# tum-vision/mono_dataset_code

Hardware: AMD Instinct MI355X
Metric: Mpix/s photometric+FOV undistort, 1280x1024 gray (higher is better)
Workload: dtype f32

## Files before the change

### mono_dataset_code_amd/build.py

```python
import os
import shutil
import subprocess
import time
import sys

PKG = os.path.dirname(os.path.abspath(__file__))
ROOT = os.path.dirname(PKG)
CSRC = os.path.join(PKG, "csrc")
HOST = os.path.join(CSRC, "host")
INC = os.path.join(ROOT, "include")
EIGEN_STUB = os.path.join(INC, "mono_dataset_code", "compat")

LIB_HIP = os.path.join(PKG, "libmdc_hip.so")
LIB_HOST = os.path.join(PKG, "libmdc_host.so")

HIP_SOURCES = [os.path.join(CSRC, f) for f in ("mdc_kernels.hip", "mdc_vcal.hip", "mdc_jpeg.hip", "mdc_capi.hip", "mdc_plan.hip", "mdc_host_calls.hip",
                                                "mdc_pipeline.hip", "mdc_placement.hip", "mdc_rcal.hip")]
HIP_DEPS = HIP_SOURCES + [os.path.join(CSRC, "mdc_exports.map"), os.path.join(CSRC, "mdc_internal.h"), os.path.join(CSRC, "mdc_ctx.h"), os.path.join(CSRC, "mdc_build_config.h"), os.path.join(CSRC, "fov_point_model.h"), os.path.join(CSRC, "minmax_first.h"), os.path.join(CSRC, "placement_classes.h"), os.path.join(CSRC, "xcd_placement.h"), os.path.join(INC, "mdc_hip.h")]
HOST_SOURCES = [os.path.join(HOST, f) for f in (
    "fov_undistorter.cpp", "photometric_undistorter.cpp", "gray_png.cpp", "host_device.cpp", "mdc_host_capi.cpp",
    "image_codecs.cpp", "image_codecs_png.cpp", "image_codecs_jpeg.cpp", "image_codecs_jpeg_stream.cpp", "zip_reader.cpp", "image_pool.cpp", "frame_source.cpp", "decode_pool.cpp",
    "prefetch_cache.cpp", "device_lanes.cpp", "batch_run.cpp", "dataset_reader.cpp")]
HOST_DEPS = HOST_SOURCES + [os.path.join(HOST, "mdc_host_exports.map"), os.path.join(HOST, "gray_png.h"), os.path.join(HOST, "host_device.h"),
                            os.path.join(HOST, "image_codecs.h"), os.path.join(HOST, "image_codecs_internal.h"), os.path.join(HOST, "image_codecs_jpeg.h"), os.path.join(HOST, "zip_reader.h"),
                            os.path.join(HOST, "frame_source.h"), os.path.join(HOST, "decode_pool.h"), os.path.join(HOST, "prefetch_cache.h"),
                            os.path.join(HOST, "device_lanes.h"), os.path.join(HOST, "batch_run.h"), os.path.join(CSRC, "png_inflate_core.h"),
                            os.path.join(INC, "mono_dataset_code", "BenchmarkDatasetReader.h"),
                            os.path.join(INC, "mdc_hip.h"), os.path.join(INC, "mdc_host.h"), os.path.join(INC, "mdc_lens.h"),
                            os.path.join(INC, "mdc_lensinv.h"), os.path.join(CSRC, "lens_inverse_model.h"),
                            os.path.join(CSRC, "lens_point_model.h"), os.path.join(CSRC, "fov_point_model.h"),
                            os.path.join(INC, "mono_dataset_code", "FOVUndistorter.h"),
                            os.path.join(INC, "mono_dataset_code", "PhotometricUndistorter.h"),
                            os.path.join(INC, "mono_dataset_code", "ExposureImage.h"),
                            os.path.join(INC, "mono_dataset_code", "MdcBind.h")]

HIP_FLAGS = ["--offload-arch=gfx950", "-O3", "-std=c++17", "-ffp-contract=off", "-fPIC", "-shared",
             "-fno-fast-math", "-fvisibility=hidden", "-fvisibility-inlines-hidden", "-Wall", "-Wno-unused-function"]
HOST_FLAGS = ["-O2", "-std=c++11", "-ffp-contract=off", "-fPIC", "-shared", "-fvisibility=hidden", "-fvisibility-inlines-hidden", "-Wall"]
HOST_EXPORT_MAP = os.path.join(HOST, "mdc_host_exports.map")
EXPORT_MAP = os.path.join(CSRC, "mdc_exports.map")
RECIPE = os.path.abspath(__file__)


def _stale(target, deps):
    if not os.path.exists(target):
        return True
    t = os.path.getmtime(target)
    return any(os.path.getmtime(d) > t for d in deps)


def _run(cmd):
    r = subprocess.run(cmd, stdout=subprocess.PIPE, stderr=subprocess.STDOUT, text=True)
    if r.returncode != 0:
        sys.stderr.write(r.stdout)
        raise RuntimeError("build failed: " + " ".join(cmd))
    return r.stdout


def hipcc():
    for c in (os.environ.get("HIPCC"), shutil.which("hipcc"), "/opt/rocm/bin/hipcc"):
        if c and os.path.exists(c):
            return c
    raise RuntimeError("hipcc not found")


def eigen_include():
    for d in ("/usr/include/eigen3", "/usr/local/include/eigen3"):
        if os.path.exists(os.path.join(d, "Eigen", "Core")):
            return d
    return EIGEN_STUB

# ... 382 lines not shown
```

### mono_dataset_code_amd/csrc/mdc_capi.hip

```cpp
#include "mdc_ctx.h"

using namespace mdc;


namespace mdc {

static thread_local std::string g_create_err;
static thread_local std::string t_err, t_err_other;
static thread_local const mdc_ctx* t_err_ctx = nullptr;

int fail(mdc_ctx* c, int code, const char* fmt, ...) {
  char buf[512];
  va_list ap;
  va_start(ap, fmt);
  vsnprintf(buf, sizeof buf, fmt, ap);
  va_end(ap);
  if (c) {
    {
      std::lock_guard<std::mutex> lk(c->err_mu);
      c->err = buf;
    }
    t_err = buf;
    t_err_ctx = c;
  } else {
// ... 898 lines not shown
  if (n < 0 || (n > 0 && (!d_vignette || !d_out)) || ((uintptr_t)d_out & 1) || ((uintptr_t)d_vignette & 3))
    return fail(c, MDC_ERR_ARG, "mdc_vcal_vignette_u16_device: bad argument");
  ReadLock lk(c->mu);
  DeviceGuard dg(c->device);
  MDC_HIP(c, launch_vcal_vignette_u16(d_vignette, n, d_out, (hipStream_t)stream));
  return MDC_OK;
} MDC_CATCH(c)

int mdc_vcal_solve_device(mdc_ctx* c, const float* d_images, const float* d_p2x, const float* d_p2y, int n_images, int w, int h,
                          int n_plane, float* d_plane_color, float* d_vignette_factor, int max_iterations, int outlier_th,
                          double* er_out, void* stream) try {
  if (!c) return MDC_ERR_ARG;
  if (!d_plane_color || !d_vignette_factor || max_iterations < 0 || outlier_th < 0 || outlier_th > 46340)
    return fail(c, MDC_ERR_ARG, "mdc_vcal_solve_device: bad argument");
  if (max_iterations == 0) return MDC_OK;
  mdc_vcal_index* index = nullptr;
  int rc = mdc_vcal_index_create(c, d_images, d_p2x, d_p2y, n_images, w, h, n_plane, stream, &index);
  if (rc != MDC_OK) return rc;
  ReadLock lk(c->mu);
  DeviceGuard dg(c->device);
  hipStream_t s = (hipStream_t)stream;
  float *d_ff = nullptr, *d_fc = nullptr, *d_tt = nullptr, *d_ct = nullptr;
  double* d_er = nullptr;
  const size_t plane_bytes = (size_t)std::max(n_plane, 1) * sizeof(float), img_bytes = (size_t)w * h * sizeof(float);
  const size_t er_bytes = (size_t)max_iterations * 4 * sizeof(double);
  auto done = [&](int code) {
    (void)hipStreamSynchronize(s);
    for (void* p : {(void*)d_ff, (void*)d_fc, (void*)d_tt, (void*)d_ct, (void*)d_er}) (void)hipFree(p);
    mdc_vcal_index_destroy(index);
    return code;
  };
#define MDC_SOLVE(call_)                                                  \
  do {                                                                    \
    hipError_t e_ = (call_);                                              \
    if (e_ != hipSuccess) return done(fail(c, MDC_ERR_HIP, "%s: %s", #call_, hipGetErrorString(e_))); \
  } while (0)
  MDC_SOLVE(hipMalloc(&d_ff, plane_bytes));
  MDC_SOLVE(hipMalloc(&d_fc, plane_bytes));
  MDC_SOLVE(hipMalloc(&d_tt, img_bytes));
  MDC_SOLVE(hipMalloc(&d_ct, img_bytes));
  MDC_SOLVE(hipMalloc(&d_er, er_bytes));
  for (int it = 0; it < max_iterations; it++) {
    const int oth2 = it < max_iterations / 2 ? 10000 * 10000 : outlier_th * outlier_th;
    MDC_SOLVE(launch_vcal_plane_step(d_images, d_p2x, d_p2y, n_images, w, h, n_plane, d_plane_color, d_vignette_factor, oth2, d_ff,
                                     d_fc, d_er + 4 * it, s));
    MDC_SOLVE(mdc::launch_vcal_vignette_step_indexed(index->ix, d_plane_color, d_vignette_factor, oth2, d_tt, d_ct, d_er + 4 * it + 2,
                                                     c->d_vcal_max + (c->vcal_max_next++ % mdc_ctx::kVcalMaxWords), s));
  }
  if (er_out) MDC_SOLVE(hipMemcpyAsync(er_out, d_er, er_bytes, hipMemcpyDeviceToHost, s));
#undef MDC_SOLVE
  return done(MDC_OK);
} MDC_CATCH(c)

int mdc_tune_device(mdc_ctx* c, const uint8_t* d_in, float* d_out, int64_t nframes, unsigned flags, void* stream,
                    mdc_tune_result* result) try {
  if (!c) return MDC_ERR_ARG;
  if (!d_in || !d_out || nframes <= 0) return fail(c, MDC_ERR_ARG, "mdc_tune_device: bad argument");
  WriteLock lk(c->mu);
  DeviceGuard dg(c->device);
  if (!(flags & MDC_RECTIFY) || !c->valid_remap) return fail(c, MDC_ERR_STATE, "mdc_tune_device: needs a remap and MDC_RECTIFY");
  hipStream_t s = (hipStream_t)stream;
  static const TileShape shapes[] = {{128, 16}, {64, 32}, {128, 32}};
  static const int fpbs[] = {32, 64, 96, 128};
  hipEvent_t e0, e1;
  MDC_HIP(c, hipEventCreate(&e0));
  MDC_HIP(c, hipEventCreate(&e1));
  float best = 1e30f;
  int bw = 0, bh = 0, bf = 0, tried = 0;
  int rc = MDC_OK;
  const int caller_fpb = c->opt_fpb;
  for (const TileShape& sh : shapes) {
    c->opt_tile_w = sh.w;
    c->opt_tile_h = sh.h;
    if (hipDeviceSynchronize() != hipSuccess) {
      rc = fail(c, MDC_ERR_HIP, "mdc_tune_device: hipDeviceSynchronize failed");
      break;
    }
    if ((rc = plan_tiles(c)) != MDC_OK) break;
    if (!c->plan[0].tiled) continue;
    for (int fpb : fpbs) {
      c->opt_fpb = fpb;
      float ms[5];
      bool ok = true;
      for (int k = 0; k < 7 && ok; k++) {
        if (k >= 2) ok = hipEventRecord(e0, s) == hipSuccess;
        ok = ok && enqueue_process(c, d_in, d_out, nframes, flags, s) == MDC_OK;
        if (k >= 2) ok = ok && hipEventRecord(e1, s) == hipSuccess && hipEventSynchronize(e1) == hipSuccess &&
                         hipEventElapsedTime(&ms[k - 2], e0, e1) == hipSuccess;
      }
      if (!ok) continue;
      std::sort(ms, ms + 5);
      tried++;
      if (ms[2] < best) {
        best = ms[2];
        bw = sh.w;
        bh = sh.h;
        bf = fpb;
      }
    }
  }
  (void)hipEventDestroy(e0);
  (void)hipEventDestroy(e1);
  (void)hipDeviceSynchronize();
  c->opt_tile_w = bw;
  c->opt_tile_h = bh;
  c->opt_fpb = caller_fpb;
  c->tuned_fpb = bf;
  c->tuned_min_frames = bf ? std::max<int64_t>(nframes / 4, (int64_t)bf * 8) : 0;
  const int rc2 = plan_tiles(c);
  if (rc == MDC_OK) rc = rc2;
  if (result) {
    result->tile_w = bw;
    result->tile_h = bh;
    result->frames_per_block = bf;
    result->ms = tried ? best : 0.f;
    result->candidates = tried;
  }
  return rc;
} MDC_CATCH(c)

int mdc_tune_placement_device(mdc_ctx* c, const uint8_t* const* d_in, int n_in, float* const* d_out, int n_out, int64_t nframes, unsigned flags,
                              void* stream, int* best_in, int* best_out, float* ms_out) try {
  if (!c) return MDC_ERR_ARG;
  if (!d_in || !d_out || n_in < 1 || n_out < 1 || (int64_t)n_in * n_out > 256 || nframes <= 0 || !best_in || !best_out)
    return fail(c, MDC_ERR_ARG, "mdc_tune_placement_device: bad argument");
  for (int k = 0; k < n_in; k++)
    if (!d_in[k]) return fail(c, MDC_ERR_ARG, "mdc_tune_placement_device: input candidate %d is NULL", k);
  for (int k = 0; k < n_out; k++)
    if (!d_out[k]) return fail(c, MDC_ERR_ARG, "mdc_tune_placement_device: output candidate %d is NULL", k);
  ReadLock lk(c->mu);
  DeviceGuard dg(c->device);
  hipStream_t s = (hipStream_t)stream;
  hipEvent_t e0, e1;
  MDC_HIP(c, hipEventCreate(&e0));
  if (hipEventCreate(&e1) != hipSuccess) {
    (void)hipEventDestroy(e0);
    return fail(c, MDC_ERR_HIP, "hipEventCreate failed");
  }
  int rc = MDC_OK, bi = 0, bo = 0;
  float best = 1e30f;
  for (int i = 0; i < n_in && rc == MDC_OK; i++)
    for (int j = 0; j < n_out && rc == MDC_OK; j++) {
      float ms[5] = {0, 0, 0, 0, 0};
      for (int k = 0; k < 7 && rc == MDC_OK; k++) {
        bool ok = k < 2 || hipEventRecord(e0, s) == hipSuccess;
        if (ok) rc = enqueue_process(c, d_in[i], d_out[j], nframes, flags, s);
        if (rc != MDC_OK) break;
        if (k >= 2) ok = ok && hipEventRecord(e1, s) == hipSuccess && hipEventSynchronize(e1) == hipSuccess && hipEventElapsedTime(&ms[k - 2], e0, e1) == hipSuccess;
        if (!ok) rc = fail(c, MDC_ERR_HIP, "mdc_tune_placement_device: timing a launch failed");
      }
      if (rc != MDC_OK) break;
      std::sort(ms, ms + 5);
      if (ms_out) ms_out[(size_t)i * n_out + j] = ms[2];
      if (ms[2] < best) {
        best = ms[2];
        bi = i;
        bo = j;
      }
    }
  (void)hipStreamSynchronize(s);
  (void)hipEventDestroy(e0);
  (void)hipEventDestroy(e1);
  *best_in = bi;
  *best_out = bo;
  return rc;
} MDC_CATCH(c)

int mdc_describe_launch(mdc_ctx* c, unsigned flags, int pyramid_levels, char* buf, size_t cap) try {
// ... 158 lines not shown
```

### mono_dataset_code_amd/csrc/mdc_ctx.h

```cpp
#pragma once
#include "../../include/mdc_hip.h"
#include "mdc_internal.h"

#include <algorithm>
#include <atomic>
#include <chrono>
#include <cmath>
#include <condition_variable>
#include <cstdarg>
#include <cstdio>
#include <cstdlib>
#include <cstring>
#include <limits>
#include <map>
#include <mutex>
#include <new>
#include <shared_mutex>
#include <string>
#include <vector>

struct mdc_ctx {
  int device = 0;
  std::shared_timed_mutex mu;
  mutable std::mutex err_mu;
// ... 103 lines not shown
  std::atomic<unsigned> vcal_max_next{0};

};
using ReadLock = std::shared_lock<std::shared_timed_mutex>;
using WriteLock = std::unique_lock<std::shared_timed_mutex>;

namespace mdc {

int fail(mdc_ctx* c, int code, const char* fmt, ...);

#define MDC_HIP(c, call)                                                                      \
  do {                                                                                        \
    hipError_t e_ = (call);                                                                   \
    if (e_ != hipSuccess) return fail((c), MDC_ERR_HIP, "%s: %s", #call, hipGetErrorString(e_)); \
  } while (0)

struct DeviceGuard {
  int prev = -1;
  explicit DeviceGuard(int dev) {
    if (hipGetDevice(&prev) != hipSuccess) prev = -1;
    if (prev != dev) (void)hipSetDevice(dev);
    else prev = -1;
  }
  ~DeviceGuard() {
    if (prev >= 0) (void)hipSetDevice(prev);
  }
};

#define MDC_CATCH(c_)                                                                    \
  catch (const std::bad_alloc&) {                                                        \
    return fail((c_), MDC_ERR_NOMEM, "out of host memory");                              \
  }                                                                                      \
  catch (const std::exception& e_) {                                                     \
    return fail((c_), MDC_ERR_HIP, "unexpected exception: %s", e_.what());               \
  }                                                                                      \
  catch (...) {                                                                          \
    return fail((c_), MDC_ERR_HIP, "unexpected exception");                              \
  }

void normalise(const mdc_ctx* c, unsigned flags, bool& g, bool& v, bool& o);
const float* lut_for(const mdc_ctx* c, bool g, bool o);
int frames_per_block(const mdc_ctx* c, int64_t nframes, int blocks_per_group, int target_wgs = 4800);
TilePlan tile_plan(const mdc_ctx* c, int which);
RemapArgs remap_args(const mdc_ctx* c, const float* lut, const float* vinv);
int enqueue_process(mdc_ctx* c, const uint8_t* d_in, float* d_out, int64_t nframes, unsigned flags, hipStream_t s, float* const* pyr = nullptr,
                    bool* pyr_done = nullptr);
int enqueue_pyramid_gradients(mdc_ctx* c, const uint8_t* d_in, float* d_base, int levels, float* const* d_levels, float* const* d_dI,
                              float* const* d_abs_squared_grad, int64_t nframes, unsigned flags, int chunk_frames, hipStream_t s);
int enqueue_undistort_f32(mdc_ctx* c, const float* d_in, float* d_out, int64_t nframes, hipStream_t s);
DistortModel distort_model(const mdc_fov_model* f);

int plan_tiles(mdc_ctx* c);
void free_plan(mdc_ctx* c);

void maybe_pin(mdc_ctx* c, int role, const void* p, size_t bytes);
void unpin_all(mdc_ctx* c);
const void* device_view_raw(const mdc_ctx* c, const void* p, size_t bytes);
template <class T>
T* device_view(const mdc_ctx* c, T* p, size_t bytes) {
  return (T*)device_view_raw(c, (const void*)p, bytes);
}
bool one_host_allocation(const void* p, size_t bytes);
int ensure_stage(mdc_ctx* c, mdc_ctx::HostSlot* h, size_t in_bytes, size_t out_bytes);

struct SlotLease {
  mdc_ctx* c;
  mdc_ctx::HostSlot* s = nullptr;
  explicit SlotLease(mdc_ctx* ctx, bool wait = true);
  bool in_flight = true;
  void drained() { in_flight = false; }
  ~SlotLease();
  SlotLease(const SlotLease&) = delete;
  SlotLease& operator=(const SlotLease&) = delete;
};

}
```

### mono_dataset_code_amd/csrc/mdc_internal.h

```cpp
#pragma once
#include <hip/hip_runtime.h>
#include <stdint.h>

#include "fov_point_model.h"
#include "mdc_build_config.h"
#include "xcd_placement.h"

namespace mdc {

struct TileShape {
  int w, h;
};
constexpr TileShape kTileShapes[] = {{64, 16}, {64, 32}, {64, 60}, {64, 64}, {128, 16}, {128, 32}};
constexpr bool tile_shape_ok(int w, int h) {
  for (const TileShape& t : kTileShapes)
    if (t.w == w && t.h == h) return true;
  return false;
}
constexpr int tile_rpt(int w, int h) { return w >= 320 ? 8 : 4; }
constexpr int tile_threads(int w, int h) { return w * h / tile_rpt(w, h); }
constexpr int kTileMaxChunks = 3;
constexpr int kTileMaxChunksF32 = 4;
constexpr int kLutRep = MDC_EXP_LUT_REP;
constexpr uint32_t kOutside = 0xfffffff0u;

struct RemapArgs {
  const float* lut;
  const float* vinv;
  const float* rx;
  const float* ry;
  int in_w, in_h, out_w, out_h;
};

struct TilePlan {
  const uint32_t* d_chunks;
  const int* d_nch;
  const uint32_t* d_taps;
  const int* d_order;
  int n_blocks;
  int n_tiles, tiles_x;
  int tile_w;
  int tile_h;
  int chunk_cap;
  int win_bytes;
  int nbuf;
  bool has_black;
  bool interleave;
  bool taper = true;
  bool rotate = false;
};

constexpr int kStripTileW = 128, kStripTileH = 8;
constexpr int kStripChunkCap = 128;
constexpr int kStripWaves = MDC_EXP_STRIP_WAVES;
struct StripPlan {
  const uint32_t* d_chunks;
  const int* d_nch;
  const uint32_t* d_taps;
  const int* d_order;
  int n_blocks, n_tiles, tiles_x;
  int win_bytes;
  int passes;
  int nbuf;
  bool interleave;
  bool rotate = false;
};
#if MDC_EXP_STRIP_FAKE_GRAD
extern float* g_fake_grad_dI;
extern float* g_fake_grad_abs;
#endif
hipError_t launch_remap_strip_u8(const uint8_t* d_in, float* d_out, const RemapArgs& a, const StripPlan& p, int64_t nframes, int fpb,
                                 hipStream_t s, float* d_l1 = nullptr, float* d_l2 = nullptr, float* d_l3 = nullptr);
size_t strip_lds_bytes(int win_bytes, int nbuf, int waves);

hipError_t launch_unmap(const uint8_t* d_in, float* d_out, const float* d_lut, const float* d_vinv, int64_t npix,
                        int64_t nframes, int fpb, hipStream_t s);

hipError_t launch_remap_gather_u8(const uint8_t* d_in, float* d_out, const RemapArgs& a, int64_t nframes, int fpb,
                                  hipStream_t s);
hipError_t launch_remap_gather_f32(const float* d_in, float* d_out, const RemapArgs& a, int64_t nframes, int fpb,
                                   hipStream_t s);
hipError_t launch_remap_tiled_u8(const uint8_t* d_in, float* d_out, const RemapArgs& a, const TilePlan& p,
                                 int64_t nframes, int fpb, hipStream_t s, float* d_l1 = nullptr, float* d_l2 = nullptr,
                                 float* d_l3 = nullptr);
hipError_t launch_remap_tiled_f32(const float* d_in, float* d_out, const RemapArgs& a, const TilePlan& p,
                                  int64_t nframes, int fpb, hipStream_t s);
size_t tiled_lds_bytes(int win_bytes, int nbuf, bool lut = true);
size_t tiled_pyramid_lds_bytes(int tile_w, int tile_h);
constexpr size_t kLdsPerCU = 160 * 1024;

hipError_t launch_prefetch_rows(const uint8_t* d_frames, int64_t frame_bytes, int row_pitch, int x0, int x1, int y0, int y1, int64_t nframes,
                                uint32_t* d_sink, hipStream_t s);

hipError_t launch_pyramid_level(const float* d_src, float* d_dst, int w, int h, int64_t nframes, hipStream_t s);

hipError_t launch_distort_points(float* d_x, float* d_y, int64_t n, const DistortModel& m, hipStream_t s);

hipError_t launch_vcal_plane_step(const float* d_images, const float* d_p2x, const float* d_p2y, int n, int wI, int hI, int np,
                                  float* d_plane_color, const float* d_vig, int oth2, float* d_ff, float* d_fc, double* d_er,
                                  hipStream_t s);
hipError_t launch_vcal_vignette_step(const float* d_images, const float* d_p2x, const float* d_p2y, int n, int wI, int hI, int np,
                                     const float* d_plane_color, float* d_vig, int oth2, float* d_tt, float* d_ct, double* d_er,
                                     unsigned* d_max_bits, hipStream_t s);

struct VcalIndex;
hipError_t vcal_index_build(const float* d_images, const float* d_p2x, const float* d_p2y, int n, int wI, int hI, int np,
                            hipStream_t s, VcalIndex** out);
void vcal_index_free(VcalIndex* ix);
long long vcal_index_bytes(const VcalIndex* ix);
long long vcal_index_entries(const VcalIndex* ix);
hipError_t launch_vcal_vignette_step_indexed(const VcalIndex* ix, const float* d_plane_color, float* d_vig, int oth2, float* d_tt,
                                             float* d_ct, double* d_er, unsigned* d_max_bits, hipStream_t s);

hipError_t launch_vcal_scale_images(float* d_images, int n, int64_t npix, float mean_exposure, const float* d_exposure, hipStream_t s);
hipError_t launch_vcal_gradient_mask(float* d_images, int n, int wI, int hI, int max_abs_grad, hipStream_t s);
hipError_t launch_vcal_mask_coords(float* d_x, float* d_y, int64_t n, int wI, int hI, hipStream_t s);
hipError_t launch_vcal_plane_coords(const float* d_corners, float* d_hk, int n, int gw, int gh, float facw, float fach,
                                    const DistortModel* m, int wI, int hI, float* d_p2x, float* d_p2y, hipStream_t s);
hipError_t launch_vcal_smooth(const float* d_vig, int wI, int hI, float* d_tt, float* d_ct, hipStream_t s);
hipError_t launch_vcal_plot_plane(const float* d_plane, long long n, uint8_t* d_rgb, float* range_host, hipStream_t s);
hipError_t launch_vcal_vignette_u16(const float* d_vignette, int64_t n, uint16_t* d_out, hipStream_t s);

hipError_t launch_jpeg_huffman(const void* d_streams, int64_t stream_stride, void* d_records, int64_t record_bytes, int w, int h, int blocks_w,
                               int blocks_rows, int64_t nframes, int* d_status, hipStream_t s, unsigned kinds = 7u, void* d_scratch = nullptr);
size_t jpeg_huffman_scratch_bytes(int64_t nframes);
int jpeg_huffman_segments(int64_t nframes);
hipError_t launch_jpeg_idct(const void* d_records, int64_t record_bytes, uint8_t* d_frames, int w, int h, int blocks_w, int blocks_rows,
                            int64_t nframes, hipStream_t s);

hipError_t launch_gradients(const float* d_level, float* d_dI, float* d_abs2, int w, int h, int64_t nframes, hipStream_t s);
hipError_t launch_gradients_levels(int n_levels, const float* const* d_src, float* const* d_dI, float* const* d_abs2, const int* w,
                                   const int* h, int64_t nframes, hipStream_t s);

}
```

### mono_dataset_code_amd/csrc/mdc_kernels.hip

```cpp
#include "mdc_internal.h"

namespace mdc {

namespace {

constexpr int kLutBytes = 256 * kLutRep * 4;
#if MDC_DEBUG_BOUNDS
#define MDC_CHECK(cond)               \
  do {                                \
    if (!(cond)) __builtin_trap();    \
  } while (0)
#else
#define MDC_CHECK(cond) \
  do {                  \
  } while (0)
#endif

typedef float f32x4 __attribute__((ext_vector_type(4)));

template <int NT>
__device__ __forceinline__ void fill_lut(float* s_lut, const float* __restrict__ lut, int tid) {
  constexpr int N = 256 * (kLutRep / 4);
  constexpr int IT = (N + NT - 1) / NT;
  float v[IT];
// ... 450 lines not shown
#else
    stage_window<R, NT>(stg, in_bytes, w[D], goff, wave, rw);
    if (f + D < last) stg += in_step;
#endif
#if MDC_EXP_TIMING
    const unsigned long long t1 = exp_now();
#endif
    float res[RPT];
#if MDC_EXP_PAD_VALU
    {
      int pad_v = tid;
#pragma unroll
      for (int q = 0; q < MDC_EXP_PAD_VALU; q++) asm volatile("v_add_u32 %0, %0, %0" : "+v"(pad_v));
    }
#endif
    tile_compute<VIG, BLACK, F32, LEAN, ((LEAN || PYR) ? 2 : 4), RPT>(t, w[0], my_lut, dst, out_bytes, row_bytes, res, win_bytes);
    if constexpr (PYR)
      pyramid_levels12(t, res, py, f_first + (long long)f * fstep, l1_bytes, l2_bytes, s_pyr + (f & 1) * G * L2W + pyr_slot,
                       tid & 63);
    dst += out_step;
#if MDC_EXP_TIMING
    const unsigned long long t2 = exp_now();
    if (PYR && pyr_all_levels) frame_wait_only<D, R, 6>(rw);
    else frame_wait_only<D, R, RPT>(rw);
    const unsigned long long t3 = exp_now();
    asm volatile("s_barrier" ::: "memory");
    const unsigned long long t4 = exp_now();
    tp[0] += t1 - t0;
    tp[1] += t2 - t1;
    tp[2] += t3 - t2;
    tp[3] += t4 - t3;
#else
    if (D > 1 && f < D - 1) wait_vm_barrier<RPT>();
    else if (PYR && pyr_all_levels) frame_barrier<D, R, 6>(rw);
    else frame_barrier<D, R, RPT>(rw);
#endif
    lds_u8_ptr x = w[0];
#pragma unroll
    for (int i = 0; i < D; i++) w[i] = w[i + 1];
    w[D] = x;
  }
  if (PYR) pyramid_level3<G, TW>(py, f_first + (long long)last * fstep, l3_bytes, s_pyr + (last & 1) * G * L2W, p3byte, tid - (NT - 64));
#if MDC_EXP_TIMING
  if ((tid & 63) == 0 && (wave == 0 || wave == 5) && blockIdx.x % 41 == 3 && blockIdx.y % 7 == 2)
    printf("TIMING block %d,%d wave %d frames %d cycles/frame: issue %.0f compute+stores %.0f vmwait %.0f barrier %.0f total %.0f\n",
           (int)blockIdx.x, (int)blockIdx.y, wave, nframes, (double)tp[0] / nframes, (double)tp[1] / nframes, (double)tp[2] / nframes,
           (double)tp[3] / nframes, (double)(exp_now() - t_begin) / nframes);
#endif
}

template <bool VIG, bool BLACK, bool PYR, bool F32, int TW, int NT, int NBUF>
__global__ __launch_bounds__(NT, (NT >= 960 ? 8 : NT == 640 ? 5 : NT == 512 ? (kLutRep < 32 ? 8 : 6) : 4)) void remap_tiled_kernel(
    const uint8_t* __restrict__ in, float* __restrict__ out, RemapArgs a, TilePlan p, PyramidOut py, int nframes, int fpb,
    int interleave, int taper_full, int taper_r) {
  constexpr int RPT = tile_rpt(TW, 0);
  extern __shared__ __attribute__((aligned(1024))) unsigned char smem[];
  float* s_lut = reinterpret_cast<float*>(smem);
  lds_u8_ptr s_win = (lds_u8_ptr)smem + (F32 ? 0 : kLutBytes);

  const int tile = p.d_order[xcd_table_entry((int)blockIdx.x, (int)blockIdx.y, p.rotate)];
  if (tile < 0) return;
  const int fstep = interleave ? (int)gridDim.y : 1;
  int f0 = interleave ? (int)blockIdx.y : (int)blockIdx.y * fpb;
  int nf = interleave ? (nframes - f0 + fstep - 1) / fstep : min(nframes, f0 + fpb) - f0;
  if (!interleave && taper_r > 0 && (int)blockIdx.y >= taper_full) {
    const int k = (int)blockIdx.y - taper_full;
    const int lvl = min(k / taper_r, 2);
    const int size = fpb >> (lvl + 1);
    f0 = taper_full * fpb + taper_r * (fpb - (fpb >> lvl)) + (k - lvl * taper_r) * size;
    nf = min(nframes, f0 + size) - f0;
  }
  if (nf <= 0) return;

  const int tid = threadIdx.x;
  const int lane_x = tid % TW;
  const int row0 = (tid / TW) * RPT;
  const int ox = (tile % p.tiles_x) * TW + lane_x;
  constexpr int kTileRows = NT * RPT / TW;
  constexpr bool LEAN = (NT >= 960 && (NBUF != 2 || BLACK || PYR || F32)) || RPT > 4;
  const int oy0 = (tile / p.tiles_x) * kTileRows + row0;

  const int nch = p.d_nch[tile];
  constexpr int RMAX = F32 ? kTileMaxChunksF32 : kTileMaxChunks;
  const uint32_t* chunks = p.d_chunks + (size_t)tile * (RMAX * NT);
  uint32_t goff[RMAX];
#pragma unroll
  for (int k = 0; k < RMAX; k++) goff[k] = chunks[tid + k * NT];

  float xx[RPT], yy[RPT];
  uint32_t tp[RPT];
#pragma unroll
  for (int j = 0; j < RPT; j++) {
    const bool inside = (ox < a.out_w) && (oy0 + j < a.out_h);
    const int oidx = inside ? (oy0 + j) * a.out_w + ox : 0;
    xx[j] = a.rx[oidx];
    yy[j] = a.ry[oidx];
    tp[j] = p.d_taps[oidx];
  }
  if (!F32) fill_lut<NT>(s_lut, a.lut, tid);
  lds_f32_ptr my_lut = (lds_f32_ptr)s_lut + (tid & (kLutRep - 1));

  TileThread<RPT> t;
#pragma unroll
  for (int j = 0; j < RPT; j++) {
    const int oy = oy0 + j;
    const bool inside = (ox < a.out_w) && (oy < a.out_h);
    const int oidx = oy * a.out_w + ox;
    if (LEAN) {
      if (j == 0) t.obyte[0] = ox < a.out_w ? (uint32_t)oidx * 4u : kOutsideLean;
    } else {
      t.obyte[j] = inside ? (uint32_t)oidx * 4u : kOutside;
    }
    if (!inside) {
      xx[j] = yy[j] = -1.f;
      tp[j] = 0;
    }
    if (PYR && j == 0)
      t.p1byte = (uint32_t)(((oy >> 1) + (lane_x & 1)) * (a.out_w >> 1) + (ox >> 1)) * 4u;
    if (PYR && j == 0) t.p2byte = (lane_x & 3) ? kOutside : (uint32_t)((oy >> 2) * (a.out_w >> 2) + (ox >> 2)) * 4u;
    t.black[j] = xx[j] < 0;
    t.bl[j] = bilin_of(t.black[j] ? 0.f : xx[j], t.black[j] ? 0.f : yy[j]);
    t.fx[j] = (t.black[j] ? 0.f : xx[j]) - (float)t.bl[j].xi;
    t.fy[j] = (t.black[j] ? 0.f : yy[j]) - (float)t.bl[j].yi;
    t.tap[j] = tp[j];
// ... 439 lines not shown

inline int ceil_div(long long a, long long b) { return (int)((a + b - 1) / b); }

}

size_t tiled_lds_bytes(int win_bytes, int nbuf, bool lut) { return (lut ? (size_t)kLutBytes : 0) + (size_t)nbuf * win_bytes; }
size_t tiled_pyramid_lds_bytes(int tile_w, int tile_h) { return (size_t)2 * (tile_h / 4) * (tile_w / 4) * sizeof(float); }

hipError_t launch_unmap(const uint8_t* d_in, float* d_out, const float* d_lut, const float* d_vinv, int64_t npix,
                        int64_t nframes, int fpb, hipStream_t s) {
  if (nframes <= 0 || npix <= 0) return hipSuccess;
  const int groups = ceil_div(nframes, fpb);
  const bool vec = (npix % 4 == 0) && ((reinterpret_cast<uintptr_t>(d_in) & 3) == 0);
  if (vec) {
    dim3 grid(ceil_div(npix, 4096), groups);
    if (d_vinv) unmap_xpose_kernel<true><<<grid, 256, 0, s>>>(d_in, d_out, d_lut, d_vinv, npix, (int)nframes, fpb);
    else unmap_xpose_kernel<false><<<grid, 256, 0, s>>>(d_in, d_out, d_lut, d_vinv, npix, (int)nframes, fpb);
  } else {
    dim3 grid(ceil_div(npix, 256), groups);
    if (d_vinv) unmap_scalar_kernel<true><<<grid, 256, 0, s>>>(d_in, d_out, d_lut, d_vinv, npix, (int)nframes, fpb);
    else unmap_scalar_kernel<false><<<grid, 256, 0, s>>>(d_in, d_out, d_lut, d_vinv, npix, (int)nframes, fpb);
  }
  return hipGetLastError();
}

hipError_t launch_remap_gather_u8(const uint8_t* d_in, float* d_out, const RemapArgs& a, int64_t nframes, int fpb,
                                  hipStream_t s) {
  if (nframes <= 0) return hipSuccess;
  dim3 grid(ceil_div((long long)a.out_w * a.out_h, 256), ceil_div(nframes, fpb));
  if (a.vinv) remap_gather_u8_kernel<true><<<grid, 256, 0, s>>>(d_in, d_out, a, (int)nframes, fpb);
  else remap_gather_u8_kernel<false><<<grid, 256, 0, s>>>(d_in, d_out, a, (int)nframes, fpb);
  return hipGetLastError();
}

hipError_t launch_remap_gather_f32(const float* d_in, float* d_out, const RemapArgs& a, int64_t nframes, int fpb,
                                   hipStream_t s) {
  if (nframes <= 0) return hipSuccess;
  dim3 grid(ceil_div((long long)a.out_w * a.out_h, 256), ceil_div(nframes, fpb));
  remap_gather_f32_kernel<<<grid, 256, 0, s>>>(d_in, d_out, a, (int)nframes, fpb);
  return hipGetLastError();
}

struct TiledLaunch {
  const uint8_t* d_in;
  float* d_out;
  RemapArgs a;
  TilePlan p;
  PyramidOut py;
  int64_t nframes;
  int fpb;
  hipStream_t s;
};

static int taper_groups(int64_t nframes, int fpb, int taper_r, int* full) {
  *full = 0;
  if (taper_r <= 0) return (int)ceil_div(nframes, fpb);
  const int64_t tail = (int64_t)taper_r * (fpb / 2 + fpb / 4);
  *full = (int)((nframes - tail) / fpb);
  const int64_t rest = nframes - (int64_t)*full * fpb - tail;
  return *full + 2 * taper_r + (int)ceil_div(rest, fpb / 8);
}

template <bool VIG, bool BLACK, bool PYR, bool F32, int TW, int NT, int NBUF>
static hipError_t launch_tiled_variant(const TiledLaunch& l) {
  const size_t lds = tiled_lds_bytes(l.p.win_bytes, NBUF, !F32) + (PYR ? tiled_pyramid_lds_bytes(l.p.tile_w, l.p.tile_h) : 0);
  const int resident = 256 * (int)std::max<size_t>(1, std::min<size_t>(2048 / NT, kLdsPerCU / std::max<size_t>(lds, 1)));
  int taper_r = std::max(2, (resident + l.p.n_blocks / 2) / std::max(1, l.p.n_blocks));
  if (!l.p.taper || l.p.interleave || l.fpb % 8 != 0 || l.fpb < 16 || l.nframes < (int64_t)l.fpb * (4 * taper_r)) taper_r = 0;
  int taper_full = 0;
  dim3 grid(l.p.n_blocks, taper_groups(l.nframes, l.fpb, taper_r, &taper_full));
  if (lds > 64 * 1024) {
    hipError_t e = hipFuncSetAttribute(reinterpret_cast<const void*>(&remap_tiled_kernel<VIG, BLACK, PYR, F32, TW, NT, NBUF>),
                                       hipFuncAttributeMaxDynamicSharedMemorySize, (int)lds);
    if (e != hipSuccess) return e;
  }
  remap_tiled_kernel<VIG, BLACK, PYR, F32, TW, NT, NBUF><<<grid, NT, lds, l.s>>>(l.d_in, l.d_out, l.a, l.p, l.py, (int)l.nframes, l.fpb,
                                                                                 l.p.interleave ? 1 : 0, taper_full, taper_r);
  return hipGetLastError();
}

template <bool VIG, bool BLACK, bool PYR, bool F32, int TW, int NT>
static hipError_t launch_tiled_buf(const TiledLaunch& l) {
  constexpr int RPT = tile_rpt(TW, 0);
  switch (l.p.nbuf) {
    case 2:
      if constexpr (RPT == 4) return launch_tiled_variant<VIG, BLACK, PYR, F32, TW, NT, 2>(l);
      break;
    case 3: return launch_tiled_variant<VIG, BLACK, PYR, F32, TW, NT, 3>(l);
    case 4:
      if constexpr (NT <= 512) return launch_tiled_variant<VIG, BLACK, PYR, F32, TW, NT, 4>(l);
      break;
  }
  return hipErrorInvalidValue;
}

template <bool VIG, bool BLACK, bool PYR, bool F32>
static hipError_t launch_tiled_shape(const TiledLaunch& l) {
  switch (l.p.tile_w * 1000 + l.p.tile_h) {
    case 64016: return launch_tiled_buf<VIG, BLACK, PYR, F32, 64, 256>(l);
    case 64032: return launch_tiled_buf<VIG, BLACK, PYR, F32, 64, 512>(l);
    case 64060:
      if constexpr (!PYR) return launch_tiled_buf<VIG, BLACK, false, F32, 64, 960>(l);
      break;
    case 64064:
      if constexpr (!PYR) return launch_tiled_buf<VIG, BLACK, false, F32, 64, 1024>(l);
      break;
    case 128016: return launch_tiled_buf<VIG, BLACK, PYR, F32, 128, 512>(l);
    case 128032:
      if constexpr (!PYR) return launch_tiled_buf<VIG, BLACK, false, F32, 128, 1024>(l);
      break;
  }
  return hipErrorInvalidValue;
}

template <bool VIG, bool BLACK>
static hipError_t launch_tiled_nt(const TiledLaunch& l) {
  const bool pyr = l.py.l1 || l.py.l2 || l.py.l3;
  return pyr ? launch_tiled_shape<VIG, BLACK, true, false>(l) : launch_tiled_shape<VIG, BLACK, false, false>(l);
}

size_t strip_lds_bytes(int win_bytes, int nbuf, int waves) {
  return (size_t)waves * ((4 + nbuf) * win_bytes + kStripPad) + kStripLutBytes
#if MDC_EXP_STRIP_FAKE_GRAD
         + (size_t)waves * 1536
#endif
      ;
}
template <bool VIG, bool PYR, int NBUF, int P>
static hipError_t launch_strip_variant(const uint8_t* d_in, float* d_out, const RemapArgs& a, const StripPlan& p, const PyramidOut& py,
                                       int64_t nframes, int fpb, hipStream_t s) {
// ... 108 lines not shown
```

Before: 3.886 million.

## Generalize tail taper for small frame counts and harden tile autotuner selection

Moves the tail-taper schedule into a shared header. The new version adapts the half- and quarter-size group counts to the frame budget, so tapering now also applies when there are only a few frames, which the old code excluded. The autotuner keeps each candidate tile plan alive, waits until timings settle, and re-times the finalists over several rounds. It only moves off the default when another candidate beats it by more than the measured spread. This adds tuning time and more blocks in the tail, in exchange for better load balance on the last wave and less noisy selection.

```diff
diff --git a/mono_dataset_code_amd/build.py b/mono_dataset_code_amd/build.py
--- a/mono_dataset_code_amd/build.py
+++ b/mono_dataset_code_amd/build.py
@@ -16,7 +16,7 @@
 
 HIP_SOURCES = [os.path.join(CSRC, f) for f in ("mdc_kernels.hip", "mdc_vcal.hip", "mdc_jpeg.hip", "mdc_capi.hip", "mdc_plan.hip", "mdc_host_calls.hip",
                                                 "mdc_pipeline.hip", "mdc_placement.hip", "mdc_rcal.hip")]
-HIP_DEPS = HIP_SOURCES + [os.path.join(CSRC, "mdc_exports.map"), os.path.join(CSRC, "mdc_internal.h"), os.path.join(CSRC, "mdc_ctx.h"), os.path.join(CSRC, "mdc_build_config.h"), os.path.join(CSRC, "fov_point_model.h"), os.path.join(CSRC, "minmax_first.h"), os.path.join(CSRC, "placement_classes.h"), os.path.join(CSRC, "xcd_placement.h"), os.path.join(INC, "mdc_hip.h")]
+HIP_DEPS = HIP_SOURCES + [os.path.join(CSRC, "mdc_exports.map"), os.path.join(CSRC, "mdc_internal.h"), os.path.join(CSRC, "mdc_ctx.h"), os.path.join(CSRC, "mdc_build_config.h"), os.path.join(CSRC, "fov_point_model.h"), os.path.join(CSRC, "minmax_first.h"), os.path.join(CSRC, "placement_classes.h"), os.path.join(CSRC, "xcd_placement.h"), os.path.join(CSRC, "tail_taper.h"), os.path.join(INC, "mdc_hip.h")]
 HOST_SOURCES = [os.path.join(HOST, f) for f in (
     "fov_undistorter.cpp", "photometric_undistorter.cpp", "gray_png.cpp", "host_device.cpp", "mdc_host_capi.cpp",
     "image_codecs.cpp", "image_codecs_png.cpp", "image_codecs_jpeg.cpp", "image_codecs_jpeg_stream.cpp", "zip_reader.cpp", "image_pool.cpp", "frame_source.cpp", "decode_pool.cpp",
diff --git a/mono_dataset_code_amd/csrc/mdc_capi.hip b/mono_dataset_code_amd/csrc/mdc_capi.hip
--- a/mono_dataset_code_amd/csrc/mdc_capi.hip
+++ b/mono_dataset_code_amd/csrc/mdc_capi.hip
@@ -974,6 +974,21 @@
   return done(MDC_OK);
 } MDC_CATCH(c)
 
+namespace {
+constexpr int kTuneRounds = 5;
+struct TuneCand {
+  int plan, fpb;
+  float coarse;
+  std::vector<float> rounds;
+  float median() const {
+    std::vector<float> r = rounds;
+    std::sort(r.begin(), r.end());
+    return r.empty() ? coarse : r[r.size() / 2];
+  }
+  float spread() const { return rounds.empty() ? 0.f : *std::max_element(rounds.begin(), rounds.end()) - *std::min_element(rounds.begin(), rounds.end()); }
+};
+}
+
 int mdc_tune_device(mdc_ctx* c, const uint8_t* d_in, float* d_out, int64_t nframes, unsigned flags, void* stream,
                     mdc_tune_result* result) try {
   if (!c) return MDC_ERR_ARG;
@@ -984,46 +999,92 @@
   hipStream_t s = (hipStream_t)stream;
   static const TileShape shapes[] = {{128, 16}, {64, 32}, {128, 32}};
   static const int fpbs[] = {32, 64, 96, 128};
+  constexpr int kLongFpb = 128;
+  constexpr int kShapes = sizeof shapes / sizeof shapes[0];
   hipEvent_t e0, e1;
   MDC_HIP(c, hipEventCreate(&e0));
-  MDC_HIP(c, hipEventCreate(&e1));
-  float best = 1e30f;
-  int bw = 0, bh = 0, bf = 0, tried = 0;
+  if (hipEventCreate(&e1) != hipSuccess) {
+    (void)hipEventDestroy(e0);
+    return fail(c, MDC_ERR_HIP, "hipEventCreate failed");
+  }
+  mdc_ctx::SrcPlan held[kShapes];
+  std::vector<TuneCand> cands;
   int rc = MDC_OK;
   const int caller_fpb = c->opt_fpb;
-  for (const TileShape& sh : shapes) {
-    c->opt_tile_w = sh.w;
-    c->opt_tile_h = sh.h;
+  auto median5 = [&](int warm, float* med) {
+    float ms[5] = {0, 0, 0, 0, 0};
+    bool ok = true;
+    for (int k = 0; k < warm + 5 && ok; k++) {
+      if (k >= warm) ok = hipEventRecord(e0, s) == hipSuccess;
+      ok = ok && enqueue_process(c, d_in, d_out, nframes, flags, s) == MDC_OK;
+      if (k >= warm) ok = ok && hipEventRecord(e1, s) == hipSuccess && hipEventSynchronize(e1) == hipSuccess &&
+                          hipEventElapsedTime(&ms[k - warm], e0, e1) == hipSuccess;
+    }
+    std::sort(ms, ms + 5);
+    *med = ms[2];
+    return ok;
+  };
+  for (int k = 0; k < kShapes; k++) {
+    c->opt_tile_w = shapes[k].w;
+    c->opt_tile_h = shapes[k].h;
     if (hipDeviceSynchronize() != hipSuccess) {
       rc = fail(c, MDC_ERR_HIP, "mdc_tune_device: hipDeviceSynchronize failed");
       break;
     }
-    if ((rc = plan_tiles(c)) != MDC_OK) break;
-    if (!c->plan[0].tiled) continue;
+    if (k > 0) c->plan[0] = mdc_ctx::SrcPlan();
+    if ((rc = plan_tiles(c)) != MDC_OK) {
+      free_src_plan(c->plan[0]);
+      break;
+    }
+    held[k] = c->plan[0];
+    if (!held[k].tiled) continue;
+    const int round = tiled_round_groups(held[k].tile_w, held[k].tile_h, tiled_lds_bytes(held[k].win_bytes, held[k].nbuf, true), held[k].n_blocks);
+    c->opt_fpb = 128;
+    float prev = 0.f, cur = 0.f;
+    bool settling = median5(0, &prev);
+    for (float spent = 5.f * prev; settling && spent < 50.f; spent += 5.f * cur, prev = cur)
+      settling = median5(0, &cur) && std::fabs(cur - prev) > 0.01f * cur;
     for (int fpb : fpbs) {
+      if (fpb > kLongFpb && (nframes + fpb - 1) / fpb < 3 * (int64_t)round) continue;
       c->opt_fpb = fpb;
-      float ms[5];
-      bool ok = true;
-      for (int k = 0; k < 7 && ok; k++) {
-        if (k >= 2) ok = hipEventRecord(e0, s) == hipSuccess;
-        ok = ok && enqueue_process(c, d_in, d_out, nframes, flags, s) == MDC_OK;
-        if (k >= 2) ok = ok && hipEventRecord(e1, s) == hipSuccess && hipEventSynchronize(e1) == hipSuccess &&
-                         hipEventElapsedTime(&ms[k - 2], e0, e1) == hipSuccess;
+      TuneCand t{k, fpb, 0.f, {}};
+      if (median5(2, &t.coarse)) cands.push_back(t);
+    }
+  }
+  const int tried = (int)cands.size();
+  int pick = -1;
+  if (rc == MDC_OK && tried > 0) {
+    c->opt_fpb = 0;
+    const int auto_fpb = frames_per_block(c, nframes, held[cands[0].plan].n_blocks);
+    int incumbent = 0;
+    float best = cands[0].coarse;
+    for (int i = 0; i < tried; i++) {
+      best = std::min(best, cands[i].coarse);
+      if (cands[i].plan == cands[0].plan && std::abs(cands[i].fpb - auto_fpb) < std::abs(cands[incumbent].fpb - auto_fpb)) incumbent = i;
+    }
+    std::vector<int> finalists;
+    for (int i = 0; i < tried; i++)
+      if (i == incumbent || cands[i].coarse <= 1.02f * best) finalists.push_back(i);
+    bool ok = true;
+    for (int r = 0; r < kTuneRounds && ok && finalists.size() > 1; r++)
+      for (int i : finalists) {
+        c->plan[0] = held[cands[i].plan];
+        c->opt_fpb = cands[i].fpb;
+        float med = 0.f;
+        if (!(ok = median5(0, &med))) break;
+        cands[i].rounds.push_back(med);
       }
-      if (!ok) continue;
-      std::sort(ms, ms + 5);
-      tried++;
-      if (ms[2] < best) {
-        best = ms[2];
-        bw = sh.w;
-        bh = sh.h;
-        bf = fpb;
-      }
-    }
+    if (!ok) rc = fail(c, MDC_ERR_HIP, "mdc_tune_device: timing a launch failed");
+    pick = incumbent;
+    for (int i : finalists)
+      if (ok && cands[pick].median() - cands[i].median() > cands[pick].spread()) pick = i;
   }
   (void)hipEventDestroy(e0);
   (void)hipEventDestroy(e1);
   (void)hipDeviceSynchronize();
+  c->plan[0] = mdc_ctx::SrcPlan();
+  for (mdc_ctx::SrcPlan& h : held) free_src_plan(h);
+  const int bw = pick >= 0 ? shapes[cands[pick].plan].w : 0, bh = pick >= 0 ? shapes[cands[pick].plan].h : 0, bf = pick >= 0 ? cands[pick].fpb : 0;
   c->opt_tile_w = bw;
   c->opt_tile_h = bh;
   c->opt_fpb = caller_fpb;
@@ -1035,7 +1096,7 @@
     result->tile_w = bw;
     result->tile_h = bh;
     result->frames_per_block = bf;
-    result->ms = tried ? best : 0.f;
+    result->ms = pick >= 0 ? cands[pick].median() : 0.f;
     result->candidates = tried;
   }
   return rc;
diff --git a/mono_dataset_code_amd/csrc/mdc_ctx.h b/mono_dataset_code_amd/csrc/mdc_ctx.h
--- a/mono_dataset_code_amd/csrc/mdc_ctx.h
+++ b/mono_dataset_code_amd/csrc/mdc_ctx.h
@@ -179,6 +179,7 @@
 
 int plan_tiles(mdc_ctx* c);
 void free_plan(mdc_ctx* c);
+void free_src_plan(mdc_ctx::SrcPlan& pl);
 
 void maybe_pin(mdc_ctx* c, int role, const void* p, size_t bytes);
 void unpin_all(mdc_ctx* c);
diff --git a/mono_dataset_code_amd/csrc/mdc_internal.h b/mono_dataset_code_amd/csrc/mdc_internal.h
--- a/mono_dataset_code_amd/csrc/mdc_internal.h
+++ b/mono_dataset_code_amd/csrc/mdc_internal.h
@@ -4,6 +4,7 @@
 
 #include "fov_point_model.h"
 #include "mdc_build_config.h"
+#include "tail_taper.h"
 #include "xcd_placement.h"
 
 namespace mdc {
@@ -88,6 +89,7 @@
 size_t tiled_lds_bytes(int win_bytes, int nbuf, bool lut = true);
 size_t tiled_pyramid_lds_bytes(int tile_w, int tile_h);
 constexpr size_t kLdsPerCU = 160 * 1024;
+int tiled_round_groups(int tile_w, int tile_h, size_t lds_bytes, int n_blocks);
 
 hipError_t launch_prefetch_rows(const uint8_t* d_frames, int64_t frame_bytes, int row_pitch, int x0, int x1, int y0, int y1, int64_t nframes,
                                 uint32_t* d_sink, hipStream_t s);
diff --git a/mono_dataset_code_amd/csrc/mdc_kernels.hip b/mono_dataset_code_amd/csrc/mdc_kernels.hip
--- a/mono_dataset_code_amd/csrc/mdc_kernels.hip
+++ b/mono_dataset_code_amd/csrc/mdc_kernels.hip
@@ -526,7 +526,7 @@
 template <bool VIG, bool BLACK, bool PYR, bool F32, int TW, int NT, int NBUF>
 __global__ __launch_bounds__(NT, (NT >= 960 ? 8 : NT == 640 ? 5 : NT == 512 ? (kLutRep < 32 ? 8 : 6) : 4)) void remap_tiled_kernel(
     const uint8_t* __restrict__ in, float* __restrict__ out, RemapArgs a, TilePlan p, PyramidOut py, int nframes, int fpb,
-    int interleave, int taper_full, int taper_r) {
+    int interleave, TailTaper taper) {
   constexpr int RPT = tile_rpt(TW, 0);
   extern __shared__ __attribute__((aligned(1024))) unsigned char smem[];
   float* s_lut = reinterpret_cast<float*>(smem);
@@ -535,15 +535,8 @@
   const int tile = p.d_order[xcd_table_entry((int)blockIdx.x, (int)blockIdx.y, p.rotate)];
   if (tile < 0) return;
   const int fstep = interleave ? (int)gridDim.y : 1;
-  int f0 = interleave ? (int)blockIdx.y : (int)blockIdx.y * fpb;
-  int nf = interleave ? (nframes - f0 + fstep - 1) / fstep : min(nframes, f0 + fpb) - f0;
-  if (!interleave && taper_r > 0 && (int)blockIdx.y >= taper_full) {
-    const int k = (int)blockIdx.y - taper_full;
-    const int lvl = min(k / taper_r, 2);
-    const int size = fpb >> (lvl + 1);
-    f0 = taper_full * fpb + taper_r * (fpb - (fpb >> lvl)) + (k - lvl * taper_r) * size;
-    nf = min(nframes, f0 + size) - f0;
-  }
+  int f0 = (int)blockIdx.y;
+  const int nf = interleave ? (nframes - f0 + fstep - 1) / fstep : tail_taper_range((int)blockIdx.y, nframes, fpb, taper, &f0);
   if (nf <= 0) return;
 
   const int tid = threadIdx.x;
@@ -1089,30 +1082,24 @@
   hipStream_t s;
 };
 
-static int taper_groups(int64_t nframes, int fpb, int taper_r, int* full) {
-  *full = 0;
-  if (taper_r <= 0) return (int)ceil_div(nframes, fpb);
-  const int64_t tail = (int64_t)taper_r * (fpb / 2 + fpb / 4);
-  *full = (int)((nframes - tail) / fpb);
-  const int64_t rest = nframes - (int64_t)*full * fpb - tail;
-  return *full + 2 * taper_r + (int)ceil_div(rest, fpb / 8);
+int tiled_round_groups(int tile_w, int tile_h, size_t lds_bytes, int n_blocks) {
+  const int resident = 256 * (int)std::max<size_t>(1, std::min<size_t>(2048 / tile_threads(tile_w, tile_h), kLdsPerCU / std::max<size_t>(lds_bytes, 1)));
+  return std::max(2, (resident + n_blocks / 2) / std::max(1, n_blocks));
 }
 
 template <bool VIG, bool BLACK, bool PYR, bool F32, int TW, int NT, int NBUF>
 static hipError_t launch_tiled_variant(const TiledLaunch& l) {
   const size_t lds = tiled_lds_bytes(l.p.win_bytes, NBUF, !F32) + (PYR ? tiled_pyramid_lds_bytes(l.p.tile_w, l.p.tile_h) : 0);
-  const int resident = 256 * (int)std::max<size_t>(1, std::min<size_t>(2048 / NT, kLdsPerCU / std::max<size_t>(lds, 1)));
-  int taper_r = std::max(2, (resident + l.p.n_blocks / 2) / std::max(1, l.p.n_blocks));
-  if (!l.p.taper || l.p.interleave || l.fpb % 8 != 0 || l.fpb < 16 || l.nframes < (int64_t)l.fpb * (4 * taper_r)) taper_r = 0;
-  int taper_full = 0;
-  dim3 grid(l.p.n_blocks, taper_groups(l.nframes, l.fpb, taper_r, &taper_full));
+  const bool tapered = l.p.taper && !l.p.interleave;
+  const TailTaper taper = tail_taper(l.nframes, l.fpb, tapered ? tiled_round_groups(l.p.tile_w, l.p.tile_h, lds, l.p.n_blocks) : 0);
+  dim3 grid(l.p.n_blocks, tail_taper_groups(l.nframes, l.fpb, taper));
   if (lds > 64 * 1024) {
     hipError_t e = hipFuncSetAttribute(reinterpret_cast<const void*>(&remap_tiled_kernel<VIG, BLACK, PYR, F32, TW, NT, NBUF>),
                                        hipFuncAttributeMaxDynamicSharedMemorySize, (int)lds);
     if (e != hipSuccess) return e;
   }
   remap_tiled_kernel<VIG, BLACK, PYR, F32, TW, NT, NBUF><<<grid, NT, lds, l.s>>>(l.d_in, l.d_out, l.a, l.p, l.py, (int)l.nframes, l.fpb,
-                                                                                 l.p.interleave ? 1 : 0, taper_full, taper_r);
+                                                                                 l.p.interleave ? 1 : 0, taper);
   return hipGetLastError();
 }
 
diff --git a/mono_dataset_code_amd/csrc/tail_taper.h b/mono_dataset_code_amd/csrc/tail_taper.h
--- /dev/null
+++ b/mono_dataset_code_amd/csrc/tail_taper.h
@@ -0,0 +1,59 @@
+#pragma once
+#include <stdint.h>
+
+#if defined(__HIPCC__)
+#define MDC_TAPER_HD __host__ __device__ __forceinline__
+#else
+#define MDC_TAPER_HD inline
+#endif
+
+namespace mdc {
+
+struct TailTaper {
+  int full;
+  int r1, r2;
+};
+
+MDC_TAPER_HD TailTaper tail_taper(int64_t nframes, int fpb, int round) {
+  TailTaper t = {0, 0, 0};
+  if (round <= 0 || fpb < 16 || fpb % 8 != 0 || nframes < 2 * (int64_t)fpb) return t;
+  const int64_t half = fpb / 2, quarter = fpb / 4, budget = nframes / 2;
+  if (budget < round * quarter) {
+    t.r2 = (int)(nframes / quarter);
+  } else {
+    const int64_t room = (budget - round * quarter) / half;
+    t.r2 = round;
+    t.r1 = (int)(room < round ? room : round);
+  }
+  t.full = (int)((nframes - t.r1 * half - t.r2 * quarter) / fpb);
+  return t;
+}
+
+MDC_TAPER_HD int tail_taper_groups(int64_t nframes, int fpb, TailTaper t) {
+  if (nframes <= 0) return 0;
+  if (t.r1 + t.r2 == 0) return (int)((nframes + fpb - 1) / fpb);
+  const int eighth = fpb / 8;
+  const int64_t rest = nframes - (int64_t)t.full * fpb - (int64_t)t.r1 * (fpb / 2) - (int64_t)t.r2 * (fpb / 4);
+  return t.full + t.r1 + t.r2 + (int)((rest + eighth - 1) / eighth);
+}
+
+MDC_TAPER_HD int tail_taper_range(int y, int nframes, int fpb, TailTaper t, int* f0) {
+  int size = fpb;
+  *f0 = y * fpb;
+  if (t.r1 + t.r2 > 0 && y >= t.full) {
+    const int k = y - t.full, base = t.full * fpb;
+    if (k < t.r1) {
+      size = fpb / 2;
+      *f0 = base + k * size;
+    } else if (k < t.r1 + t.r2) {
+      size = fpb / 4;
+      *f0 = base + t.r1 * (fpb / 2) + (k - t.r1) * size;
+    } else {
+      size = fpb / 8;
+      *f0 = base + t.r1 * (fpb / 2) + t.r2 * size * 2 + (k - t.r1 - t.r2) * size;
+    }
+  }
+  return (nframes < *f0 + size ? nframes : *f0 + size) - *f0;
+}
+
+}
```

Result: slower. 3.751 million (-3.5%).
